# castorini/daam

Measured on NVIDIA H100. Metric: heatmap px/s (layers x steps x tokens), higher is better.
Workload: dtype bf16

## Files before the change

### daam_b200/csrc/accumulate_mma.cu

```cuda
#include <cuda.h>

#include <mutex>
#include <type_traits>
#include <unordered_map>
#include <string>

#include "common.cuh"

namespace daam {
namespace {

constexpr int kStages = 2;
constexpr int kAccStages = 3;
constexpr int kPrefetchTiles = 6;
constexpr int kQBytes = kTilePixels * 128;
constexpr int kKBytes = kTokensPad * 128;
constexpr int kStageBytes = kQBytes + kKBytes;
constexpr int kPBytes = kTokens * kTilePixels * 4;
constexpr int kConsumers = 256;
constexpr int kThreads = kConsumers + 32;
constexpr int kThreads16 = kConsumers + 64;
constexpr int kBarBytes = 64;
constexpr int kBarBytes16 = 8 * 2 * (kStages + kAccStages);
constexpr int kSmemBytes = 1024 + kStages * kStageBytes + kAccStages * kPBytes + kBarBytes16;
constexpr int kSlabSmemBytes = kSmemBytes + kPBytes;
constexpr int kSplitStageBytes = 2 * kStageBytes;
constexpr int kSplitSmemBytes = 1024 + (kStages + 1) * kSplitStageBytes + kPBytes + kBarBytes;
static_assert(kSmemBytes <= 232448, "16-bit form exceeds the 227 KB shared-memory limit");
static_assert(kSplitSmemBytes <= 232448, "split form exceeds the 227 KB shared-memory limit");
static_assert(kSlabSmemBytes <= 232448, "16-bit second-slab form exceeds the 227 KB shared-memory limit");
constexpr int long_smem_bytes(int chunks) {
  return 1024 + kStages * (kQBytes + chunks * kKBytes) + kAccStages * kPBytes + kBarBytes16;
}
static_assert(long_smem_bytes(3) <= 232448, "16-bit long-context form exceeds the 227 KB shared-memory limit");

struct MmaParams {
  LaunchParams base;
  CUtensorMap qmap[kMaxLayersPerLaunch];
  CUtensorMap kmap[kMaxLayersPerLaunch];
  CUtensorMap amap[kMaxLayersPerLaunch];
};
struct MmaSlabParams : MmaParams {
  CUtensorMap smap[kMaxLayersPerLaunch];
  float* slab[kMaxLayersPerLaunch];
};
template <bool kSecond>
using MmaParamsT = std::conditional_t<kSecond, MmaSlabParams, MmaParams>;

__device__ __forceinline__ uint32_t smem_u32(const void* p) { return (uint32_t)__cvta_generic_to_shared(p); }

__device__ __forceinline__ void mbar_init(uint32_t bar, uint32_t count) {
  asm volatile("mbarrier.init.shared::cta.b64 [%0], %1;" ::"r"(bar), "r"(count));
}
__device__ __forceinline__ void mbar_arrive(uint32_t bar) {
  asm volatile("mbarrier.arrive.shared::cta.b64 _, [%0];" ::"r"(bar) : "memory");
}
// ... 173 lines not shown
    for (int u = 0; u < 4; ++u)
      if (off + u * stride < end) {
        float4 h, l;
        h.x = trunc_tf32(x[u].x); h.y = trunc_tf32(x[u].y); h.z = trunc_tf32(x[u].z); h.w = trunc_tf32(x[u].w);
        l.x = rna_tf32(x[u].x - h.x); l.y = rna_tf32(x[u].y - h.y);
        l.z = rna_tf32(x[u].z - h.z); l.w = rna_tf32(x[u].w - h.w);
        *reinterpret_cast<float4*>(raw + off + u * stride) = h;
        *reinterpret_cast<float4*>(lo + off + u * stride) = l;
      }
  }
}

template <bool kBf16>
__device__ __forceinline__ void wgmma_chunk_16bit(Frag& d, uint32_t a_src, uint32_t k_src) {
  wgmma_fence();
#pragma unroll
  for (int k = 0; k < 4; ++k) wgmma_16bit<kBf16>(d, wgmma_desc_sw128(a_src + 32 * k), wgmma_desc_sw128(k_src + 32 * k));
  wgmma_commit();
  wgmma_wait0();
}
template <bool kBf16, int kC>
__device__ __forceinline__ void wgmma_chunk_16bit_long(Frag (&d)[kC], uint32_t a_src, uint32_t k_src) {
  wgmma_fence();
#pragma unroll
  for (int c = 0; c < kC; ++c)
#pragma unroll
    for (int k = 0; k < 4; ++k)
      wgmma_16bit<kBf16>(d[c], wgmma_desc_sw128(a_src + 32 * k), wgmma_desc_sw128(k_src + c * kKBytes + 32 * k));
  wgmma_commit();
  wgmma_wait0();
}

__device__ __forceinline__ void griddep_wait() { asm volatile("griddepcontrol.wait;" ::: "memory"); }

template <bool kSplit, bool kChunked, int kSlab, int kC = 1>
__global__ void __launch_bounds__(kSplit ? kThreads : kThreads16, 1)
accumulate_mma_kernel(const __grid_constant__ MmaParamsT<kSlab != kSlabNone> MP) {
  static_assert(kC == 1 || (!kSplit && kSlab == kSlabNone), "long contexts: 16-bit form, plain slab mode only");
  constexpr bool kSecond = kSlab != kSlabNone;
  constexpr int kCtx = kC * kTokens;
  constexpr int kStageBytesT = kSplit ? kSplitStageBytes : kQBytes + kC * kKBytes;
  constexpr int kOperandBytes = (kSplit ? kStages + 1 : kStages) * kStageBytesT;
  constexpr int kPTiles = kSplit ? 1 : kAccStages + (kSecond ? 1 : 0);
  const LaunchParams& P = MP.base;
  extern __shared__ uint8_t smem_raw[];
  const uint32_t raw = smem_u32(smem_raw);
  const uint32_t base = (raw + 1023u) & ~1023u;
  uint8_t* gen = smem_raw + (base - raw);
  float* sP = reinterpret_cast<float*>(gen + kOperandBytes);
  const uint32_t sP_u32 = base + kOperandBytes;
  float* sS = sP + kAccStages * (kTokens * kTilePixels);
  const uint32_t sS_u32 = sP_u32 + kAccStages * kPBytes;
  const uint32_t bars = sP_u32 + kPTiles * kPBytes;
  const uint32_t full0 = bars, empty0 = bars + 8 * kStages;
  const uint32_t afull0 = bars + 16 * kStages, aempty0 = afull0 + 8 * kAccStages;

  const int warp = threadIdx.x >> 5, lane = threadIdx.x & 31;
  int first, count, stride = 1;
  if constexpr (!kChunked && !kSplit) {
    first = blockIdx.x;
    stride = gridDim.x;
    count = (P.total_tiles - (int)blockIdx.x + stride - 1) / stride;
  } else if constexpr (!kChunked) {
    const int per = P.total_tiles / gridDim.x, rem = P.total_tiles % gridDim.x;
    first = blockIdx.x * per + min((int)blockIdx.x, rem);
    count = per + ((int)blockIdx.x < rem ? 1 : 0);
  } else {
    first = tile_at_weight(P, (long long)P.total_weight * blockIdx.x / gridDim.x);
    count = tile_at_weight(P, (long long)P.total_weight * (blockIdx.x + 1) / gridDim.x) - first;
  }

  if (threadIdx.x == 0) {
#pragma unroll
    for (int s = 0; s < kStages; ++s) {
      mbar_init(full0 + 8 * s, 1);
      mbar_init(empty0 + 8 * s, kConsumers / 32);
    }
    if constexpr (!kSplit) {
#pragma unroll
      for (int s = 0; s < kAccStages; ++s) {
        mbar_init(afull0 + 8 * s, 1);
        mbar_init(aempty0 + 8 * s, 1);
      }
    }
    asm volatile("fence.mbarrier_init.release.cluster;" ::: "memory");
  }
  if (count > 0 && lane == 0 && (warp == (kSplit ? 0 : 9) || warp == 8)) {
    int li0 = 0;
    const Tile t0 = decode_tile(P, first, li0);
    if (warp != 8) {
      prefetch_tensormap(&MP.amap[t0.li]);
      if constexpr (kSecond) prefetch_tensormap(&MP.smap[t0.li]);
    } else {
      prefetch_tensormap(&MP.qmap[t0.li]);
      prefetch_tensormap(&MP.kmap[t0.li]);
    }
  }
  __syncthreads();
  if (!P.early_loads) griddep_wait();
  asm volatile("griddepcontrol.launch_dependents;" ::: "memory");

  if (warp == 9) {
    if constexpr (!kSplit) {
      if (lane == 0 && count > 0) {
        if (P.early_loads) griddep_wait();
        const uint64_t pol = l2_evict_first();
        int li = 0;
        for (int i = 0; i < count; ++i) {
          const Tile t = decode_tile(P, first + i * stride, li);
#pragma unroll
          for (int c = 0; c < kC; ++c) {
            const int n = i * kC + c;
            const int a = n % kAccStages;
            mbar_wait(aempty0 + 8 * a, ((uint32_t)(n / kAccStages) & 1u) ^ 1u);
            mbar_expect_tx(afull0 + 8 * a, kPBytes);
            tma_load_2d_hint(&MP.amap[t.li], afull0 + 8 * a, sP_u32 + a * kPBytes, t.pixel0,
                             (t.prompt * P.layer[t.li].heads + t.head) * kCtx + c * kTokens, pol);
          }
        }
      }
    }
  } else if (warp == 8) {
    if (lane == 0) {
      int li = 0, j = 0;
      for (int i = 0; i < count; ++i) {
        if (!kSplit && P.early_loads && i == (kChunked ? 1 : kStages)) {
          const uint64_t pol = l2_evict_last();
          const int end = min(count, i + kPrefetchTiles);
          int pli = 0;
          Tile prev = decode_tile(P, first + (i - 1) * stride, pli);
          for (int p = i; p < end; ++p) {
            const Tile u = decode_tile(P, first + p * stride, pli);
            const bool new_head = u.li != prev.li || u.prompt != prev.prompt || u.head != prev.head;
            const int nc = kChunked ? (P.layer[u.li].head_dim + 63) >> 6 : 1;
            for (int c = 0; c < nc; ++c) {
              tma_prefetch_4d(&MP.qmap[u.li], 64 * c, u.head, u.pixel0, u.prompt, pol);
              if (new_head)
#pragma unroll
                for (int kc = 0; kc < kC; ++kc) tma_prefetch_4d(&MP.kmap[u.li], 64 * c, u.head, kc * kTokens, u.prompt, pol);
            }
            prev = u;
          }
        }
        const Tile t = decode_tile(P, first + i * stride, li);
        const int n_chunks = kChunked ? (P.layer[t.li].head_dim + 63) >> 6 : 1;
        for (int c = 0; c < n_chunks; ++c, ++j) {
          const int s = j % kStages;
          const uint32_t ph = (uint32_t)(j / kStages) & 1u;
          mbar_wait(empty0 + 8 * s, ph ^ 1u);
          const uint32_t q_dst = base + s * kStageBytesT;
          if constexpr (kSplit) {
// ... 101 lines not shown
        f[4 * jj + 2] = l0 ? fast_exp2(fmaf(f[4 * jj + 2], sc, -mc1)) : 0.f;
        f[4 * jj + 1] = l1 ? fast_exp2(fmaf(f[4 * jj + 1], sc, -mc0)) : 0.f;
        f[4 * jj + 3] = l1 ? fast_exp2(fmaf(f[4 * jj + 3], sc, -mc1)) : 0.f;
        sum0 += f[4 * jj] + f[4 * jj + 1];
        sum1 += f[4 * jj + 2] + f[4 * jj + 3];
      }
      sum0 += __shfl_xor_sync(0xffffffffu, sum0, 1);
      sum0 += __shfl_xor_sync(0xffffffffu, sum0, 2);
      sum1 += __shfl_xor_sync(0xffffffffu, sum1, 1);
      sum1 += __shfl_xor_sync(0xffffffffu, sum1, 2);
      const float inv0 = 1.0f / sum0, inv1 = 1.0f / sum1;

      if constexpr (!kSplit) {
#pragma unroll
        for (int kc = 0; kc < kC; ++kc) {
        const int n = i * kC + kc;
        const int a = n % kAccStages;
        float* sA = sP + a * (kTokens * kTilePixels);
        const bool lowq = quad < 2;
        const int ra = lowq ? r0 : r0 + 8, rb = lowq ? r0 + 8 : r0;
        mbar_wait(afull0 + 8 * a, (uint32_t)(n / kAccStages) & 1u);
        float old[40];
#pragma unroll
        for (int jj = 0; jj < 10; ++jj) {
#pragma unroll
          for (int e = 0; e < 2; ++e) {
            const int col = 8 * jj + 2 * quad + e;
            if (col < kTokens) {
              old[4 * jj + e] = sA[col * kTilePixels + ra];
              old[4 * jj + 2 + e] = sA[col * kTilePixels + rb];
            }
          }
        }
        if constexpr (kSecond) {
          if (tid == 0 && i > 0) bulk_wait_read0();
          consumer_barrier();
        }
        const float* f = dd[kc];
#pragma unroll
        for (int jj = 0; jj < 10; ++jj) {
#pragma unroll
          for (int e = 0; e < 2; ++e) {
            const int col = 8 * jj + 2 * quad + e;
            if (col < kTokens) {
              const float pa = f[4 * jj + e] * inv0, pb = f[4 * jj + 2 + e] * inv1;
              sA[col * kTilePixels + ra] = add_ftz(old[4 * jj + e], lowq ? pa : pb);
              sA[col * kTilePixels + rb] = add_ftz(old[4 * jj + 2 + e], lowq ? pb : pa);
              if constexpr (kSecond) {
                sS[col * kTilePixels + ra] = add_ftz(0.f, lowq ? pa : pb);
                sS[col * kTilePixels + rb] = add_ftz(0.f, lowq ? pb : pa);
              }
            }
          }
        }
        fence_proxy_async();
        consumer_barrier();
        if (tid == 0) {
          tma_store_2d_hint(&MP.amap[t.li], sP_u32 + a * kPBytes, t.pixel0,
                            (t.prompt * L.heads + t.head) * kCtx + kc * kTokens, l2_evict_first());
          if constexpr (kSlab == kSlabStore)
            tma_store_2d(&MP.smap[t.li], sS_u32, t.pixel0, (t.prompt * L.heads + t.head) * kTokens);
          if constexpr (kSlab == kSlabAdd)
            tma_reduce_add_2d(&MP.smap[t.li], sS_u32, t.pixel0, (t.prompt * L.heads + t.head) * kTokens);
          bulk_commit();
          if (n > 0) {
            bulk_wait_read1();
            mbar_arrive(aempty0 + 8 * ((n - 1) % kAccStages));
          }
        }
        }
        continue;
      }

      if (i == 0 && P.early_loads) griddep_wait();

      if (tid == 0 && issued) bulk_wait_read0();
      consumer_barrier();
      const bool lowq = quad < 2;
      const bool stage_ftz = kSlab == kSlabStore && P.rmw_mode == 1;
#pragma unroll
      for (int jj = 0; jj < 10; ++jj) {
#pragma unroll
        for (int e = 0; e < 2; ++e) {
          const int col = 8 * jj + 2 * quad + e;
          if (col < kTokens) {
            float a = d[4 * jj + e] * inv0, b = d[4 * jj + 2 + e] * inv1;
            if constexpr (kSecond) {
              if (stage_ftz) { a = add_ftz(0.f, a); b = add_ftz(0.f, b); }
            }
            sP[col * kTilePixels + (lowq ? r0 : r0 + 8)] = lowq ? a : b;
            sP[col * kTilePixels + (lowq ? r0 + 8 : r0)] = lowq ? b : a;
          }
        }
      }
      if (P.rmw_mode == 1) {
        fence_proxy_async();
        consumer_barrier();
        if (tid == 0) {
          tma_reduce_add_2d(&MP.amap[t.li], sP_u32, t.pixel0, (t.prompt * L.heads + t.head) * kTokens);
          if constexpr (kSlab == kSlabStore)
            tma_store_2d(&MP.smap[t.li], sP_u32, t.pixel0, (t.prompt * L.heads + t.head) * kTokens);
          if constexpr (kSlab == kSlabAdd)
            tma_reduce_add_2d(&MP.smap[t.li], sP_u32, t.pixel0, (t.prompt * L.heads + t.head) * kTokens);
          bulk_commit();
        }
        issued = true;
      } else {
        consumer_barrier();
        const long long hw = L.hw;
        float* acc = L.acc + ((long long)(t.prompt * L.heads + t.head) * kTokens) * hw + t.pixel0;
        const int live = min(kTilePixels, L.hw - t.pixel0) >> 2;
        for (int u = tid; u < kTokens * (kTilePixels / 4); u += kConsumers) {
          const int tok = u / (kTilePixels / 4), c4 = u % (kTilePixels / 4);
          if (c4 < live) {
            float4* g = reinterpret_cast<float4*>(acc + tok * hw) + c4;
            const float4 p = reinterpret_cast<const float4*>(sP + tok * kTilePixels)[c4];
            float4 o = *g;
            o.x += p.x; o.y += p.y; o.z += p.z; o.w += p.w;
            *g = o;
            if constexpr (kSlab == kSlabStore)
              reinterpret_cast<float4*>(MP.slab[t.li] + (acc - L.acc) + tok * hw)[c4] = p;
            if constexpr (kSlab == kSlabAdd) {
              float4* r = reinterpret_cast<float4*>(MP.slab[t.li] + (acc - L.acc) + tok * hw) + c4;
              float4 ro = *r;
              ro.x += p.x; ro.y += p.y; ro.z += p.z; ro.w += p.w;
              *r = ro;
            }
          }
        }
      }
    }
    if (tid == 0 && (kSplit ? issued : count > 0)) bulk_wait_read0();
  }
}

using EncodeFn = CUresult (*)(CUtensorMap*, CUtensorMapDataType, cuuint32_t, void*, const cuuint64_t*,
                              const cuuint64_t*, const cuuint32_t*, const cuuint32_t*, CUtensorMapInterleave,
                              CUtensorMapSwizzle, CUtensorMapL2promotion, CUtensorMapFloatOOBfill);

EncodeFn get_encode() {
  static EncodeFn fn = nullptr;
  static std::once_flag once;
  std::call_once(once, [] {
    void* p = nullptr;
    cudaDriverEntryPointQueryResult q;
    if (cudaGetDriverEntryPoint("cuTensorMapEncodeTiled", &p, cudaEnableDefault, &q) == cudaSuccess &&
        q == cudaDriverEntryPointSuccess)
      fn = reinterpret_cast<EncodeFn>(p);
  });
  return fn;
}

struct MapKey {
  const void* ptr;
  long long s1, s2, s3;
  int d1, d2, d3, kind;
  bool operator==(const MapKey& o) const {
    return ptr == o.ptr && s1 == o.s1 && s2 == o.s2 && s3 == o.s3 && d1 == o.d1 && d2 == o.d2 && d3 == o.d3 &&
           kind == o.kind;
  }
};
struct MapKeyHash {
  size_t operator()(const MapKey& k) const {
    size_t h = reinterpret_cast<size_t>(k.ptr);
    auto mix = [&h](long long v) { h ^= (size_t)v + 0x9e3779b97f4a7c15ull + (h << 6) + (h >> 2); };
// ... 113 lines not shown
    set_error("the wgmma kernel takes %d-token contexts, or 154 / 231 tokens for 16-bit layers without a second slab "
              "(got %d)", kTokens, ctx);
    return DAAM_E_UNSUPPORTED;
  }
  bool chunked = false;
  for (int i = 0; i < p.n_layers; ++i) {
    const LayerParams& L = p.layer[i];
    if ((L.dtype == DAAM_F32) != split) { set_error("mixed fp32 / 16-bit layers in one wgmma pack"); return DAAM_E_INVALID; }
    if (L.tokens != ctx) { set_error("mixed context lengths in one wgmma pack"); return DAAM_E_INVALID; }
    if (int rc = make_qk_map(L.q, L.dtype, L.head_dim, L.heads, L.hw, L.n_prompts, L.qs_head, L.qs_pixel, L.qs_prompt, kTilePixels, &mp.qmap[i])) return rc;
    if (int rc = make_qk_map(L.k, L.dtype, L.head_dim, L.heads, ctx, L.n_prompts, L.ks_head, L.ks_token, L.ks_prompt, kTokensPad, &mp.kmap[i])) return rc;
    if (int rc = make_acc_map(L.acc, L.hw, L.n_prompts * L.heads * ctx, &mp.amap[i])) return rc;
    if (slabs) {
      if (int rc = make_acc_map(slabs->slab[i], L.hw, L.n_prompts * L.heads * kTokens, &mp.smap[i])) return rc;
      mp.slab[i] = slabs->slab[i];
    }
    chunked = chunked || L.head_dim > 64;
  }
  cudaError_t attr_err = cudaSuccess;
  std::call_once(g_attr_once[dev.device & 63], [&] {
    for (const MmaInstance& k : kMmaInstances)
      if (cudaError_t e = cudaFuncSetAttribute(k.fn, cudaFuncAttributeMaxDynamicSharedMemorySize, k.smem)) attr_err = e;
  });
  DAAM_CUDA_TRY(attr_err);
  pm.grid = dev.sm_count;
  if (pm.grid > p.total_tiles) pm.grid = p.total_tiles;
  pm.block = split ? kThreads : kThreads16;
  pm.variant = ctx == kTokens ? (split ? 1 : 0) | (chunked ? 2 : 0) | (mode << 2)
                              : kLongVariant0 + (chunked ? 1 : 0) + (ctx == 3 * kTokens ? 2 : 0);
  pm.second = mode != kSlabNone;
  return DAAM_OK;
}

int launch_prepared_mma(const void* prepared, cudaStream_t stream) {
  const PreparedMma& pm = *static_cast<const PreparedMma*>(prepared);
  const MmaInstance& k = kMmaInstances[pm.variant];
  cudaLaunchConfig_t cfg = {};
  cfg.gridDim = dim3(pm.grid);
  cfg.blockDim = dim3(pm.block);
  cfg.dynamicSmemBytes = k.smem;
  cfg.stream = stream;
  cudaLaunchAttribute attr[1];
  attr[0].id = cudaLaunchAttributeProgrammaticStreamSerialization;
  attr[0].val.programmaticStreamSerializationAllowed = pm.mp.base.pdl ? 1 : 0;
  cfg.attrs = attr;
  cfg.numAttrs = 1;
  const MmaParams* plain = &pm.mp;
  void* args[] = {pm.second ? (void*)&pm.mp : (void*)plain};
  DAAM_CUDA_TRY(cudaLaunchKernelExC(&cfg, k.fn, args));
  DAAM_CUDA_TRY(cudaGetLastError());
  count_launch();
  return DAAM_OK;
}

}
```

### daam_b200/_native.py

```python
from __future__ import annotations

import ctypes
import os
from typing import Optional, Sequence, Tuple

LIB_NAME = 'libdaam_b200.so'
LIB_PATH = os.path.join(os.path.dirname(os.path.abspath(__file__)), LIB_NAME)

DAAM_F32, DAAM_F16, DAAM_BF16 = 0, 1, 2
ACC_AUTO, ACC_FORCE_SIMT, ACC_FORCE_MMA = 0, 1, 2
ACC_RMW_AUTO, ACC_RMW_LDST, ACC_RMW_RED = 0x00, 0x10, 0x20
ACC_NO_PDL = 0x100
ACC_EARLY_LOADS = 0x200
ABI_VERSION = 4
E_INVALID, E_UNSUPPORTED, E_CUDA = -1, -2, -3
TOKENS = 77
CONTEXT_TOKENS = (77, 154, 231)
EXPAND_SCRATCH_FLOATS = 64
MAX_SEGMENT_WORDS = 96


def segment_scratch_floats(n_maps: int, n_words: int) -> int:
    return 64 * n_maps * n_words

# ... 6 lines not shown

SWEEP_MAX_THRESHOLDS = 64


def region_sweep_scratch_floats(n_maps: int, n_words: int, n_regions: int, n_thresholds: int, out_h: int,
                                out_w: int) -> int:
    return n_maps * n_words * (64 + (n_regions + 1) * n_thresholds)


WORD_OVERLAP_CTAS = 256


def word_overlap_scratch_floats(n_maps: int, n_words: int, out_h: int, out_w: int) -> int:
    tiles = ((out_h + 15) // 16) * ((out_w + 63) // 64)
    return n_maps * (n_words * 64 + (n_words * (n_words + 3) // 2) * min(tiles, WORD_OVERLAP_CTAS))


WORD_INSTANCES_MAX = 64


def word_instances_plane_bytes(out_h: int, out_w: int) -> int:
    return 8 * out_h * out_w + 48 * ((out_h + 1) // 2) * ((out_w + 1) // 2) + 260


def overlay_frames_bytes(n_maps: int, n_words: int, out_h: int, out_w: int) -> int:
    return (n_maps * n_words * out_h * out_w * 3 + 3) // 4 * 4


EXPORTS = ('daam_accumulate', 'daam_accumulate_steps', 'daam_accumulate_range', 'daam_attention_probs', 'daam_accumulate_probs', 'daam_finalize',
           'daam_finalize_maps', 'daam_finalize_parts', 'daam_finalize_per_key','daam_normalize_maps', 'daam_word_heat_map', 'daam_expand_as', 'daam_expand_words',
           'daam_segment_words', 'daam_region_overlap', 'daam_region_sweep', 'daam_word_overlap', 'daam_word_instances', 'daam_overlay_words', 'daam_jet_colormap',
           'daam_side_launcher_create', 'daam_side_launcher_destroy',
           'daam_side_launcher_launch', 'daam_side_launcher_join', 'daam_side_launcher_idle', 'daam_abi_version',
           'daam_last_error', 'daam_device_info', 'daam_launch_count')


class DaamLayer(ctypes.Structure):
    _fields_ = [
        ('q', ctypes.c_void_p), ('k', ctypes.c_void_p), ('acc', ctypes.c_void_p),
        ('q_stride_prompt', ctypes.c_int64), ('q_stride_pixel', ctypes.c_int64), ('q_stride_head', ctypes.c_int64),
        ('k_stride_prompt', ctypes.c_int64), ('k_stride_token', ctypes.c_int64), ('k_stride_head', ctypes.c_int64),
        ('n_prompts', ctypes.c_int32), ('heads', ctypes.c_int32), ('hw', ctypes.c_int32), ('tokens', ctypes.c_int32),
        ('head_dim', ctypes.c_int32), ('dtype', ctypes.c_int32), ('scale', ctypes.c_float),
        ('reserved', ctypes.c_int32),
    ]


class DaamKeyGroup(ctypes.Structure):
    _fields_ = [
        ('acc', ctypes.c_void_p), ('heads', ctypes.c_int32), ('h', ctypes.c_int32), ('w', ctypes.c_int32),
        ('tokens', ctypes.c_int32), ('head_sel', ctypes.c_int32), ('n_blocks', ctypes.c_int32),
    ]
    reserved = property(lambda self: self.n_blocks, lambda self, v: setattr(self, 'n_blocks', v))


class DaamMapSel(ctypes.Structure):
    _fields_ = [
        ('block_begin', ctypes.c_int32), ('block_count', ctypes.c_int32), ('n_rows', ctypes.c_int32),
        ('reserved', ctypes.c_int32), ('out', ctypes.c_void_p),
    ]


class DaamMapPart(ctypes.Structure):
    _fields_ = [
        ('group_begin', ctypes.c_int32), ('group_count', ctypes.c_int32), ('n_rows', ctypes.c_int32),
        ('reserved', ctypes.c_int32), ('out', ctypes.c_void_p),
    ]
# ... 61 lines not shown
    lib.daam_region_overlap.argtypes = [vp, i32, i32, i32, i32, ctypes.POINTER(i32), ctypes.POINTER(i32), i32, i32, i32,
                                        i32, i32, f32, vp, vp, i32, vp, vp, vp, vp]
    lib.daam_region_overlap.restype = ctypes.c_int
    lib.daam_region_sweep.argtypes = [vp, i32, i32, i32, i32, ctypes.POINTER(i32), ctypes.POINTER(i32), i32, i32, i32,
                                      i32, ctypes.POINTER(f32), i32, vp, vp, i32, vp, vp, vp, vp]
    lib.daam_region_sweep.restype = ctypes.c_int
    lib.daam_word_overlap.argtypes = [vp, i32, i32, i32, i32, ctypes.POINTER(i32), ctypes.POINTER(i32), i32, i32, i32,
                                      i32, i32, f32, vp, vp, vp, vp, vp]
    lib.daam_word_overlap.restype = ctypes.c_int
    lib.daam_word_instances.argtypes = [vp, i32, i32, i32, i32, ctypes.POINTER(i32), ctypes.POINTER(i32), i32, i32,
                                        i32, i32, f32, i32, vp, vp, vp, vp, vp, vp, vp, vp, i64, vp]
    lib.daam_word_instances.restype = ctypes.c_int
    lib.daam_overlay_words.argtypes = [vp, i32, i32, i32, i32, ctypes.POINTER(i32), ctypes.POINTER(i32), i32, i32, i32,
                                       i32, i32, f32, i32, vp, vp, i64, vp, vp, vp]
    lib.daam_overlay_words.restype = ctypes.c_int
    lib.daam_jet_colormap.argtypes = [vp]
    lib.daam_jet_colormap.restype = ctypes.c_int
    lib.daam_side_launcher_create.argtypes = [ctypes.POINTER(vp)]
    lib.daam_side_launcher_create.restype = ctypes.c_int
    lib.daam_side_launcher_destroy.argtypes = [vp]
    lib.daam_side_launcher_destroy.restype = None
    lib.daam_side_launcher_launch.argtypes = [vp, ctypes.POINTER(DaamLayer), i32, u32, vp, vp]
    lib.daam_side_launcher_launch.restype = ctypes.c_int
    lib.daam_side_launcher_join.argtypes = [vp, vp]
    lib.daam_side_launcher_join.restype = ctypes.c_int
    lib.daam_side_launcher_idle.argtypes = [vp]
    lib.daam_side_launcher_idle.restype = ctypes.c_int
    lib.daam_last_error.argtypes = []
    lib.daam_last_error.restype = ctypes.c_char_p
    lib.daam_device_info.argtypes = [ctypes.POINTER(i32)] * 3
    lib.daam_device_info.restype = ctypes.c_int
    lib.daam_launch_count.argtypes = []
    lib.daam_launch_count.restype = i64
    _lib = lib
    return lib


def _check(rc: int):
    if rc != 0:
        raise NativeError(rc, load().daam_last_error().decode('utf-8', 'replace'))


class PackedLayers:

    def __init__(self, layers: Sequence[DaamLayer]):
        self.n = len(layers)
        self.array = (DaamLayer * max(self.n, 1))(*layers)


class SideLauncher:

    def __init__(self):
        self._lib = load()
        handle = ctypes.c_void_p()
        _check(self._lib.daam_side_launcher_create(ctypes.byref(handle)))
        self._h = handle

    def launch(self, packed: 'PackedLayers', flags: int, producer_stream: int, side_stream: int):
        rc = self._lib.daam_side_launcher_launch(self._h, packed.array, packed.n, flags, producer_stream, side_stream)
        if rc != 0:
            _check(rc)

    def join(self, stream: int):
        rc = self._lib.daam_side_launcher_join(self._h, stream)
        if rc != 0:
            _check(rc)
# ... 202 lines not shown
                                      *_word_list(x, rows_per_word, out_h, out_w, absolute, threshold)[:-2],
                                      float(threshold), max_instances, vp(word_maps_ptr), vp(count_ptr), vp(area_ptr),
                                      vp(box_ptr), vp(sum_yx_ptr), vp(peak_ptr), vp(peak_yx_ptr), vp(scratch_ptr),
                                      scratch_bytes, vp(stream)))


def overlay_words(maps_ptr: int, n_maps: int, n_rows: int, x, rows_per_word: Sequence[Sequence[int]], out_h: int,
                  out_w: int, absolute: bool, threshold: Optional[float], color_normalize: bool, word_maps_ptr: int,
                  image_ptr: int, image_map_stride: int, frames_ptr: int, scratch_ptr: int, stream: int):
    _check(load().daam_overlay_words(ctypes.c_void_p(maps_ptr), n_maps, n_rows,
                                     *_word_list(x, rows_per_word, out_h, out_w, absolute, threshold),
                                     int(bool(color_normalize)), ctypes.c_void_p(word_maps_ptr),
                                     ctypes.c_void_p(image_ptr), image_map_stride, ctypes.c_void_p(frames_ptr),
                                     ctypes.c_void_p(scratch_ptr), ctypes.c_void_p(stream)))


def jet_colormap():
    import torch
    out = torch.empty((256, 3), dtype=torch.float32)
    _check(load().daam_jet_colormap(ctypes.c_void_p(out.data_ptr())))
    return out


def device_info():
    sm, major, minor = ctypes.c_int32(), ctypes.c_int32(), ctypes.c_int32()
    _check(load().daam_device_info(ctypes.byref(sm), ctypes.byref(major), ctypes.byref(minor)))
    return {'sm_count': sm.value, 'cc': (major.value, minor.value)}


def launch_count() -> int:
    return int(load().daam_launch_count())


def abi_version() -> int:
    return int(load().daam_abi_version())
```

### daam_b200/csrc/api.cu

```cuda
#include <atomic>
#include <cstdarg>
#include <cstdio>
#include <cstring>
#include <memory>
#include <mutex>
#include <vector>

#include "common.cuh"

namespace daam {

static thread_local char g_error[512] = "";
static std::atomic<long long> g_launches{0};

void set_error(const char* fmt, ...) {
  va_list ap;
  va_start(ap, fmt);
  vsnprintf(g_error, sizeof(g_error), fmt, ap);
  va_end(ap);
}

int cuda_fail(cudaError_t e, const char* what) {
  set_error("CUDA error %d (%s) in %s", (int)e, cudaGetErrorString(e), what);
  return DAAM_E_CUDA;
}

void count_launch(int n) { g_launches.fetch_add(n, std::memory_order_relaxed); }

int get_device_info(DeviceInfo* out) {
  static std::mutex mu;
  static DeviceInfo cache[64];
  int dev = 0;
  DAAM_CUDA_TRY(cudaGetDevice(&dev));
  std::lock_guard<std::mutex> lock(mu);
  if (dev < 0 || dev >= 64) { set_error("device index %d out of range", dev); return DAAM_E_CUDA; }
  if (cache[dev].device != dev) {
    cudaDeviceProp prop;
    DAAM_CUDA_TRY(cudaGetDeviceProperties(&prop, dev));
// ... 14 lines not shown
  if (in.dtype != DAAM_F32 && in.dtype != DAAM_F16 && in.dtype != DAAM_BF16) { set_error("daam_accumulate: layer %d: unknown dtype %d", index, in.dtype); return DAAM_E_INVALID; }
  if (in.tokens != kTokens && in.tokens != 2 * kTokens && in.tokens != 3 * kTokens) { set_error("daam_accumulate: layer %d: tokens = %d, only %d, %d or %d (one to three %d-token CLIP chunks) are traced", index, in.tokens, kTokens, 2 * kTokens, 3 * kTokens, kTokens); return DAAM_E_UNSUPPORTED; }
  if (in.head_dim <= 0 || in.head_dim % 8 != 0 || in.head_dim > DAAM_MAX_HEAD_DIM) { set_error("daam_accumulate: layer %d: head_dim = %d must be a multiple of 8 in (0, %d]", index, in.head_dim, DAAM_MAX_HEAD_DIM); return DAAM_E_UNSUPPORTED; }
  if (in.n_prompts <= 0 || in.heads <= 0 || in.hw <= 0) { set_error("daam_accumulate: layer %d: non-positive n_prompts/heads/hw", index); return DAAM_E_INVALID; }
  if (need_acc && reinterpret_cast<uintptr_t>(in.acc) % 16 != 0) { set_error("daam_accumulate: layer %d: acc is not 16-byte aligned", index); return DAAM_E_INVALID; }
  if (!(in.scale > 0.f)) { set_error("daam_accumulate: layer %d: scale must be positive", index); return DAAM_E_INVALID; }
  LayerParams& L = *out;
  L.q = in.q; L.k = in.k; L.acc = in.acc;
  L.qs_prompt = in.q_stride_prompt; L.qs_pixel = in.q_stride_pixel; L.qs_head = in.q_stride_head;
  L.ks_prompt = in.k_stride_prompt; L.ks_token = in.k_stride_token; L.ks_head = in.k_stride_head;
  L.n_prompts = in.n_prompts; L.heads = in.heads; L.hw = in.hw; L.head_dim = in.head_dim;
  L.dtype = in.dtype;
  L.scale_log2e = in.scale * 1.4426950408889634f;
  L.tiles_per_head = (in.hw + kTilePixels - 1) / kTilePixels;
  L.tile_begin = 0;
  const size_t es = dtype_size(in.dtype);
  auto aligned = [&](long long stride) { return (stride * (long long)es) % 16 == 0; };
  L.weight = 1;
  L.weight_begin = 0;
  L.vec_ok = reinterpret_cast<uintptr_t>(in.q) % 16 == 0 && reinterpret_cast<uintptr_t>(in.k) % 16 == 0 &&
             aligned(in.q_stride_prompt) && aligned(in.q_stride_pixel) && aligned(in.q_stride_head) &&
             aligned(in.k_stride_prompt) && aligned(in.k_stride_token) && aligned(in.k_stride_head);
  L.tokens = in.tokens;
  return DAAM_OK;
}

}

using namespace daam;

namespace daam {
namespace {

struct PlannedLaunch {
  bool is_mma = false;
  LaunchParams simt;
  SlabMode mode = kSlabNone;
  SecondSlabs slabs;
  int grid = 0;
  size_t smem = 0;
  struct MmaDeleter { void operator()(void* p) const { prepared_mma_delete(p); } };
  std::unique_ptr<void, MmaDeleter> mma;
};

struct Plan {
  std::vector<uint8_t> key;
  uint32_t flags = 0;
  int device = -1;
  SlabMode mode = kSlabNone;
  std::vector<PlannedLaunch> launches;
  uint64_t stamp = 0;
};
constexpr size_t kMaxPlans = 32;

size_t slab_bytes(const LayerParams& l) { return (size_t)l.n_prompts * l.heads * l.tokens * l.hw * sizeof(float); }

bool spans_overlap(const void* a, size_t na, const void* b, size_t nb) {
  const char *pa = static_cast<const char*>(a), *pb = static_cast<const char*>(b);
  return pa < pb + nb && pb < pa + na;
}

bool acc_overlap(const LayerParams& a, const LayerParams& b) {
  return spans_overlap(a.acc, slab_bytes(a), b.acc, slab_bytes(b));
}

const char* slab_word(SlabMode mode) { return mode == kSlabAdd ? "range" : "step"; }

int validate_second_slabs(const char* fn, const daam_layer* layers, float* const* slabs, int n_layers, SlabMode mode) {
// ... 5 lines not shown
  }
  for (int i = 0; i < n_layers; ++i) {
    if (!slabs[i]) { set_error("%s: layer %d has a null %s slab", fn, i, what); return DAAM_E_INVALID; }
    if (reinterpret_cast<uintptr_t>(slabs[i]) % 16 != 0) { set_error("%s: layer %d: the %s slab is not 16-byte aligned", fn, i, what); return DAAM_E_INVALID; }
  }
  for (int i = 0; i < n_layers; ++i) {
    const size_t n = slab_bytes(all[i]);
    for (int j = 0; j < n_layers; ++j) {
      if (spans_overlap(slabs[i], n, all[j].acc, slab_bytes(all[j]))) {
        set_error("%s: the %s slab of layer %d overlaps the accumulator of layer %d", fn, what, i, j);
        return DAAM_E_INVALID;
      }
      if (j != i && spans_overlap(slabs[i], n, slabs[j], slab_bytes(all[j]))) {
        set_error("%s: the %s slabs of layers %d and %d overlap", fn, what, i, j);
        return DAAM_E_INVALID;
      }
    }
  }
  return DAAM_OK;
}

int build_plan(const daam_layer* layers, float* const* slabs, SlabMode mode, int n_layers, uint32_t flags,
               const DeviceInfo& dev, Plan* plan) {
  const uint32_t path = flags & 3u, rmw = flags & DAAM_ACC_RMW_MASK;
  constexpr int kPacks = 7;
  LaunchParams packs[kPacks];
  SecondSlabs pack_slabs[kPacks];
  for (LaunchParams& p : packs) {
    p.n_layers = p.total_tiles = 0;
    p.rmw_mode = (rmw == DAAM_ACC_RMW_LDST) ? 0 : 1;
    p.pdl = (flags & DAAM_ACC_NO_PDL) ? 0 : 1;
    p.early_loads = (flags & DAAM_ACC_EARLY_LOADS) && p.pdl ? 1 : 0;
    p.total_weight = 0;
  }
  packs[1].early_loads = 0;
  auto close = [&](int which) -> int {
    LaunchParams& p = packs[which];
    if (p.n_layers == 0) return DAAM_OK;
    plan->launches.emplace_back();
    PlannedLaunch& l = plan->launches.back();
    l.is_mma = which != 2 && which < 5;
    const SecondSlabs* st = slabs ? &pack_slabs[which] : nullptr;
    int rc;
    if (l.is_mma) {
      l.mma.reset(prepared_mma_new());
      rc = prepare_accumulate_mma(p, st, mode, dev, l.mma.get());
    } else {
      l.simt = p;
      l.mode = mode;
      if (st) l.slabs = *st;
      rc = prepare_accumulate_simt(p, mode, dev, &l.grid, &l.smem);
    }
    p.n_layers = 0;
    p.total_tiles = 0;
    p.total_weight = 0;
    return rc;
  };
  for (int i = 0; i < n_layers; ++i) {
    LayerParams L;
    if (int rc = make_layer_params(layers[i], i, &L, true)) return rc;
    const int ctx_chunks = L.tokens / kTokens;
    const bool use_mma = path != DAAM_ACC_FORCE_SIMT && dev.cc_major == 9 && mma_supported(L) &&
                         (ctx_chunks == 1 || L.dtype != DAAM_F32);
    if (path == DAAM_ACC_FORCE_MMA && !use_mma) {
      set_error("daam_accumulate: layer %d cannot take the wgmma path (dtype %d, head_dim %d, alignment %d, hw = %d, "
                "tokens = %d, %d prompts with prompt strides q %lld / k %lld, sm_%d%d)", i, L.dtype, L.head_dim,
                L.vec_ok, L.hw, L.tokens, L.n_prompts, L.qs_prompt, L.ks_prompt, dev.cc_major, dev.cc_minor);
      return DAAM_E_UNSUPPORTED;
    }
    const int which = ctx_chunks > 1 ? (use_mma ? 1 : 3) + ctx_chunks : use_mma ? (L.dtype == DAAM_F32 ? 1 : 0) : 2;
    LaunchParams& p = packs[which];
    for (int m = 0; m < p.n_layers; ++m)
      if (acc_overlap(p.layer[m], L)) {
        if (int rc = close(which)) return rc;
        break;
      }
    L.tile_begin = p.total_tiles;
    const int n_chunks = (L.head_dim + 63) / 64;
    L.weight = which == 1 ? n_chunks : 1 + 4 * n_chunks;
    L.weight_begin = p.total_weight;
    if (slabs) pack_slabs[which].slab[p.n_layers] = slabs[i];
    p.layer[p.n_layers++] = L;
    p.total_tiles += L.tiles_per_head * L.heads * L.n_prompts;
    p.total_weight += L.tiles_per_head * L.heads * L.n_prompts * L.weight;
    if (p.n_layers == kMaxLayersPerLaunch)
      if (int rc = close(which)) return rc;
  }
  for (int which = 0; which < kPacks; ++which)
    if (int rc = close(which)) return rc;
  return DAAM_OK;
}

}
}

namespace daam {
namespace {

int accumulate_impl(const char* fn, const daam_layer* layers, float* const* slabs, SlabMode mode, int32_t n_layers,
                    uint32_t flags, void* stream_) {
  if (n_layers < 0 || (n_layers > 0 && !layers)) { set_error("%s: bad layer array", fn); return DAAM_E_INVALID; }
  if (n_layers == 0) return DAAM_OK;
  const bool with_slabs = mode != kSlabNone;
  if (with_slabs && !slabs) { set_error("%s: %s_acc is a null array", fn, slab_word(mode)); return DAAM_E_INVALID; }
  cudaStream_t stream = static_cast<cudaStream_t>(stream_);
  DeviceInfo dev;
  if (int rc = get_device_info(&dev)) return rc;

  static thread_local std::vector<std::unique_ptr<Plan>> plans;
  static thread_local uint64_t clock = 0;
  const size_t layer_bytes = sizeof(daam_layer) * (size_t)n_layers;
  const size_t slab_ptr_bytes = with_slabs ? sizeof(float*) * (size_t)n_layers : 0;
  const size_t bytes = layer_bytes + slab_ptr_bytes;
  Plan* plan = nullptr;
  for (auto& c : plans)
    if (c->key.size() == bytes && c->flags == flags && c->device == dev.device && c->mode == mode &&
        memcmp(c->key.data(), layers, layer_bytes) == 0 &&
        (!with_slabs || memcmp(c->key.data() + layer_bytes, slabs, slab_ptr_bytes) == 0)) {
      plan = c.get();
      break;
    }
  if (!plan) {
    if (with_slabs)
      if (int rc = validate_second_slabs(fn, layers, slabs, n_layers, mode)) return rc;
    std::unique_ptr<Plan> fresh(new Plan);
    fresh->key.assign(reinterpret_cast<const uint8_t*>(layers), reinterpret_cast<const uint8_t*>(layers) + layer_bytes);
    if (with_slabs)
      fresh->key.insert(fresh->key.end(), reinterpret_cast<const uint8_t*>(slabs),
                        reinterpret_cast<const uint8_t*>(slabs) + slab_ptr_bytes);
    fresh->flags = flags;
    fresh->device = dev.device;
    fresh->mode = mode;
    if (int rc = build_plan(layers, slabs, mode, n_layers, flags, dev, fresh.get())) return rc;
    if (plans.size() >= kMaxPlans) {
      size_t oldest = 0;
      for (size_t i = 1; i < plans.size(); ++i)
        if (plans[i]->stamp < plans[oldest]->stamp) oldest = i;
      plans[oldest] = std::move(fresh);
      plan = plans[oldest].get();
    } else {
      plans.push_back(std::move(fresh));
      plan = plans.back().get();
    }
  }
  plan->stamp = ++clock;
  for (const PlannedLaunch& l : plan->launches) {
    const int rc = l.is_mma ? launch_prepared_mma(l.mma.get(), stream)
                            : launch_prepared_simt(l.simt, l.mode != kSlabNone ? &l.slabs : nullptr, l.mode, l.grid,
                                                   l.smem, stream);
    if (rc) return rc;
  }
  return DAAM_OK;
}

}
}

extern "C" int daam_accumulate(const daam_layer* layers, int32_t n_layers, uint32_t flags, void* stream) {
  return accumulate_impl("daam_accumulate", layers, nullptr, kSlabNone, n_layers, flags, stream);
}

extern "C" int daam_accumulate_steps(const daam_layer* layers, float* const* step_acc, int32_t n_layers, uint32_t flags,
                                     void* stream) {
  return accumulate_impl("daam_accumulate_steps", layers, step_acc, kSlabStore, n_layers, flags, stream);
}

extern "C" int daam_accumulate_range(const daam_layer* layers, float* const* range_acc, int32_t n_layers, uint32_t flags,
                                     void* stream) {
  return accumulate_impl("daam_accumulate_range", layers, range_acc, kSlabAdd, n_layers, flags, stream);
}

struct daam_side_launcher {
  cudaEvent_t ready = nullptr, done = nullptr;
  int device = -1;
  bool launched = false;
};

extern "C" int daam_side_launcher_create(daam_side_launcher** out) {
  if (!out) { set_error("daam_side_launcher_create: null pointer"); return DAAM_E_INVALID; }
  DeviceInfo dev;
  if (int rc = get_device_info(&dev)) return rc;
  std::unique_ptr<daam_side_launcher> h(new daam_side_launcher);
  h->device = dev.device;
  DAAM_CUDA_TRY(cudaEventCreateWithFlags(&h->ready, cudaEventDisableTiming));
// ... 12 lines not shown
  delete h;
}

extern "C" int daam_side_launcher_launch(daam_side_launcher* h, const daam_layer* layers, int32_t n_layers, uint32_t flags,
                                         void* producer_stream, void* side_stream) {
  if (!h) { set_error("daam_side_launcher_launch: null launcher"); return DAAM_E_INVALID; }
  cudaStream_t producer = static_cast<cudaStream_t>(producer_stream), side = static_cast<cudaStream_t>(side_stream);
  DAAM_CUDA_TRY(cudaEventRecord(h->ready, producer));
  DAAM_CUDA_TRY(cudaStreamWaitEvent(side, h->ready, 0));
  if (int rc = daam_accumulate(layers, n_layers, flags, side_stream)) return rc;
  DAAM_CUDA_TRY(cudaEventRecord(h->done, side));
  h->launched = true;
  return DAAM_OK;
}

extern "C" int daam_side_launcher_join(daam_side_launcher* h, void* stream) {
  if (!h) { set_error("daam_side_launcher_join: null launcher"); return DAAM_E_INVALID; }
  if (h->launched) DAAM_CUDA_TRY(cudaStreamWaitEvent(static_cast<cudaStream_t>(stream), h->done, 0));
  return DAAM_OK;
}

extern "C" int daam_side_launcher_idle(daam_side_launcher* h) {
  if (!h) { set_error("daam_side_launcher_idle: null launcher"); return DAAM_E_INVALID; }
  if (!h->launched) return 1;
  const cudaError_t e = cudaEventQuery(h->done);
  if (e == cudaSuccess) return 1;
  if (e == cudaErrorNotReady) return 0;
  return cuda_fail(e, "cudaEventQuery");
}

extern "C" int daam_abi_version(void) { return DAAM_ABI_VERSION; }
extern "C" const char* daam_last_error(void) { return g_error; }
extern "C" int64_t daam_launch_count(void) { return g_launches.load(std::memory_order_relaxed); }

extern "C" int daam_device_info(int32_t* sm_count, int32_t* cc_major, int32_t* cc_minor) {
  DeviceInfo dev;
  if (int rc = get_device_info(&dev)) return rc;
  if (sm_count) *sm_count = dev.sm_count;
  if (cc_major) *cc_major = dev.cc_major;
  if (cc_minor) *cc_minor = dev.cc_minor;
  return DAAM_OK;
}
```

### daam_b200/csrc/common.cuh

```cuda
#pragma once

#include <cuda_runtime.h>
#include <cuda_bf16.h>
#include <cuda_fp16.h>
#include <stdint.h>

#include "daam_b200.h"

namespace daam {

constexpr int kTokens = DAAM_TOKENS;
constexpr int kTokensPad = 80;
constexpr int kTilePixels = 128;
constexpr int kMaxLayersPerLaunch = 32;

struct LayerParams {
  const void* q;
  const void* k;
  float* acc;
  long long qs_prompt, qs_pixel, qs_head;
  long long ks_prompt, ks_token, ks_head;
  int n_prompts, heads, hw, head_dim;
  int dtype;
  float scale_log2e;
  int tiles_per_head;
  int tile_begin;
  int vec_ok;
  int weight;
  int weight_begin;
  int tokens;
};

struct LaunchParams {
  int n_layers;
  int total_tiles;
  int rmw_mode;
  int pdl;
  int early_loads;
  int total_weight;
  LayerParams layer[kMaxLayersPerLaunch];
};

__device__ __forceinline__ float fast_exp2(float x) {
  float y;
  asm("ex2.approx.ftz.f32 %0, %1;" : "=f"(y) : "f"(x));
  return y;
}

__device__ __forceinline__ float add_ftz(float a, float b) {
  float r;
  asm("add.rn.ftz.f32 %0, %1, %2;" : "=f"(r) : "f"(a), "f"(b));
  return r;
}

struct SecondSlabs {
  float* slab[kMaxLayersPerLaunch];
};
enum SlabMode : int { kSlabNone = 0, kSlabStore = 1, kSlabAdd = 2 };

void set_error(const char* fmt, ...);
int cuda_fail(cudaError_t e, const char* what);
#define DAAM_CUDA_TRY(expr)                                        \
  do {                                                             \
    cudaError_t e_ = (expr);                                       \
    if (e_ != cudaSuccess) return ::daam::cuda_fail(e_, #expr);    \
  } while (0)

struct DeviceInfo {
  int device = -1;
  int sm_count = 0;
  int cc_major = 0, cc_minor = 0;
};
int get_device_info(DeviceInfo* out);
void count_launch(int n = 1);

int prepare_accumulate_simt(const LaunchParams& p, SlabMode mode, const DeviceInfo& dev, int* grid, size_t* smem);
int launch_prepared_simt(const LaunchParams& p, const SecondSlabs* slabs, SlabMode mode, int grid, size_t smem,
                         cudaStream_t stream);
void* prepared_mma_new();
void prepared_mma_delete(void* prepared);
int prepare_accumulate_mma(const LaunchParams& p, const SecondSlabs* slabs, SlabMode mode, const DeviceInfo& dev,
                           void* prepared);
int launch_prepared_mma(const void* prepared, cudaStream_t stream);
bool mma_supported(const LayerParams& l);

}
```

### include/daam_b200.h

```cpp
#ifndef DAAM_B200_H
#define DAAM_B200_H

#include <stdint.h>

#ifdef __cplusplus
extern "C" {
#endif

#define DAAM_ABI_VERSION 4
#define DAAM_TOKENS 77
#define DAAM_MAX_TOKENS 231
#define DAAM_MAX_HEAD_DIM 256

enum daam_status {
  DAAM_OK = 0,
  DAAM_E_INVALID = -1,
  DAAM_E_UNSUPPORTED = -2,
  DAAM_E_CUDA = -3
};

enum daam_dtype { DAAM_F32 = 0, DAAM_F16 = 1, DAAM_BF16 = 2 };

#define DAAM_ACC_AUTO        0u
#define DAAM_ACC_FORCE_SIMT  1u
// ... 109 lines not shown
#define DAAM_WORD_OVERLAP_CTAS 256
#define DAAM_WORD_OVERLAP_SCRATCH_FLOATS(n_maps, n_words, out_h, out_w)                                               \
  ((int64_t)(n_maps) * ((n_words) * 64 + ((n_words) * ((n_words) + 3) / 2) *                                         \
       ((((out_h) + 15) / 16) * (((out_w) + 63) / 64) < DAAM_WORD_OVERLAP_CTAS                                       \
            ? (((out_h) + 15) / 16) * (((out_w) + 63) / 64) : DAAM_WORD_OVERLAP_CTAS)))
int daam_word_overlap(const float* global_maps, int32_t n_maps, int32_t n_rows, int32_t map_h, int32_t map_w,
                      const int32_t* rows, const int32_t* row_begin, int32_t n_words, int32_t out_h, int32_t out_w,
                      int32_t absolute, int32_t use_threshold, float threshold, float* word_maps,
                      float* intersection, float* word_area, float* scratch, void* stream);

#define DAAM_WORD_INSTANCES_MAX 64
#define DAAM_WORD_INSTANCES_PLANE_BYTES(out_h, out_w)                                                                 \
  (8 * (int64_t)(out_h) * (out_w) + 48 * (int64_t)(((out_h) + 1) / 2) * (((out_w) + 1) / 2) + 260)
int daam_word_instances(const float* global_maps, int32_t n_maps, int32_t n_rows, int32_t map_h, int32_t map_w,
                        const int32_t* rows, const int32_t* row_begin, int32_t n_words, int32_t out_h, int32_t out_w,
                        int32_t absolute, float threshold, int32_t max_instances, float* word_maps, int32_t* count,
                        int32_t* area, int32_t* box, int64_t* sum_yx, float* peak, int32_t* peak_yx, void* scratch,
                        int64_t scratch_bytes, void* stream);

#define DAAM_OVERLAY_FRAMES_BYTES(n_maps, n_words, out_h, out_w)                                                      \
  (((int64_t)(n_maps) * (n_words) * (out_h) * (out_w) * 3 + 3) / 4 * 4)
int daam_overlay_words(const float* global_maps, int32_t n_maps, int32_t n_rows, int32_t map_h, int32_t map_w,
                       const int32_t* rows, const int32_t* row_begin, int32_t n_words, int32_t out_h, int32_t out_w,
                       int32_t absolute, int32_t use_threshold, float threshold, int32_t color_normalize,
                       float* word_maps, const uint8_t* image, int64_t image_map_stride, uint8_t* frames,
                       float* scratch, void* stream);

int daam_jet_colormap(float* out);

int daam_abi_version(void);
const char* daam_last_error(void);
int daam_device_info(int32_t* sm_count, int32_t* cc_major, int32_t* cc_minor);
int64_t daam_launch_count(void);

#ifdef __cplusplus
}
#endif
#endif
```

Before: 267.5 billion.

## Move accumulator TMA stores to a dedicated store warp with mbarrier handoff

Adds a third producer-side warp that waits on new per-stage 'filled' mbarriers and issues the TMA stores and slab stores and reductions, then frees accumulator stages. Consumers no longer run a block-wide barrier and single-thread store issue after each tile; each warp just arrives on the barrier. This aims to take store issue and bulk-wait latency off the consumer critical path. It costs an extra warp and more barriers, and adds subtle phase and ordering logic around the shared slab buffer (sfree) that could introduce races.

```diff
diff --git a/daam_b200/csrc/accumulate_mma.cu b/daam_b200/csrc/accumulate_mma.cu
--- a/daam_b200/csrc/accumulate_mma.cu
+++ b/daam_b200/csrc/accumulate_mma.cu
@@ -19,9 +19,9 @@
 constexpr int kPBytes = kTokens * kTilePixels * 4;
 constexpr int kConsumers = 256;
 constexpr int kThreads = kConsumers + 32;
-constexpr int kThreads16 = kConsumers + 64;
+constexpr int kThreads16 = kConsumers + 96;
 constexpr int kBarBytes = 64;
-constexpr int kBarBytes16 = 8 * 2 * (kStages + kAccStages);
+constexpr int kBarBytes16 = 8 * (2 * kStages + 3 * kAccStages + 1);
 constexpr int kSmemBytes = 1024 + kStages * kStageBytes + kAccStages * kPBytes + kBarBytes16;
 constexpr int kSlabSmemBytes = kSmemBytes + kPBytes;
 constexpr int kSplitStageBytes = 2 * kStageBytes;
@@ -283,6 +283,8 @@
   const uint32_t bars = sP_u32 + kPTiles * kPBytes;
   const uint32_t full0 = bars, empty0 = bars + 8 * kStages;
   const uint32_t afull0 = bars + 16 * kStages, aempty0 = afull0 + 8 * kAccStages;
+  const uint32_t afilled0 = aempty0 + 8 * kAccStages;
+  const uint32_t sfree = afilled0 + 8 * kAccStages;
 
   const int warp = threadIdx.x >> 5, lane = threadIdx.x & 31;
   int first, count, stride = 1;
@@ -310,7 +312,9 @@
       for (int s = 0; s < kAccStages; ++s) {
         mbar_init(afull0 + 8 * s, 1);
         mbar_init(aempty0 + 8 * s, 1);
-      }
+        mbar_init(afilled0 + 8 * s, kConsumers / 32);
+      }
+      mbar_init(sfree, 1);
     }
     asm volatile("fence.mbarrier_init.release.cluster;" ::: "memory");
   }
@@ -329,7 +333,52 @@
   if (!P.early_loads) griddep_wait();
   asm volatile("griddepcontrol.launch_dependents;" ::: "memory");
 
-  if (warp == 9) {
+  if (warp == 10) {
+    if constexpr (!kSplit) {
+      if (lane == 0 && count > 0) {
+        const uint64_t pol = l2_evict_first();
+        int li = 0;
+        bool held = false;
+        Tile t = decode_tile(P, first, li);
+        for (int i = 0; i < count; ++i) {
+          Tile next = t;
+          if (i + 1 < count) {
+            next = decode_tile(P, first + (i + 1) * stride, li);
+            if (next.li != t.li) {
+              prefetch_tensormap(&MP.amap[next.li]);
+              if constexpr (kSecond) prefetch_tensormap(&MP.smap[next.li]);
+            }
+          }
+          const int row = t.prompt * P.layer[t.li].heads + t.head;
+#pragma unroll
+          for (int c = 0; c < kC; ++c) {
+            const int n = i * kC + c;
+            const int a = n % kAccStages;
+            mbar_wait(afilled0 + 8 * a, (uint32_t)(n / kAccStages) & 1u);
+            tma_store_2d_hint(&MP.amap[t.li], sP_u32 + a * kPBytes, t.pixel0, row * kCtx + c * kTokens, pol);
+            if constexpr (kSlab == kSlabStore)
+              tma_store_2d(&MP.smap[t.li], sS_u32, t.pixel0, row * kTokens);
+            if constexpr (kSlab == kSlabAdd)
+              tma_reduce_add_2d(&MP.smap[t.li], sS_u32, t.pixel0, row * kTokens);
+            bulk_commit();
+            if (held) {
+              bulk_wait_read1();
+              mbar_arrive(aempty0 + 8 * ((n - 1) % kAccStages));
+              if constexpr (kSecond) mbar_arrive(sfree);
+            }
+            const int n1 = n + 1;
+            held = n1 < count * kC && mbar_try(afilled0 + 8 * (n1 % kAccStages), (uint32_t)(n1 / kAccStages) & 1u);
+            if (!held) {
+              bulk_wait_read0();
+              mbar_arrive(aempty0 + 8 * a);
+              if constexpr (kSecond) mbar_arrive(sfree);
+            }
+          }
+          t = next;
+        }
+      }
+    }
+  } else if (warp == 9) {
     if constexpr (!kSplit) {
       if (lane == 0 && count > 0) {
         if (P.early_loads) griddep_wait();
@@ -513,10 +562,8 @@
             }
           }
         }
-        if constexpr (kSecond) {
-          if (tid == 0 && i > 0) bulk_wait_read0();
-          consumer_barrier();
-        }
+        if constexpr (kSecond)
+          mbar_wait(sfree, ((uint32_t)i & 1u) ^ 1u);
         const float* f = dd[kc];
 #pragma unroll
         for (int jj = 0; jj < 10; ++jj) {
@@ -535,20 +582,8 @@
           }
         }
         fence_proxy_async();
-        consumer_barrier();
-        if (tid == 0) {
-          tma_store_2d_hint(&MP.amap[t.li], sP_u32 + a * kPBytes, t.pixel0,
-                            (t.prompt * L.heads + t.head) * kCtx + kc * kTokens, l2_evict_first());
-          if constexpr (kSlab == kSlabStore)
-            tma_store_2d(&MP.smap[t.li], sS_u32, t.pixel0, (t.prompt * L.heads + t.head) * kTokens);
-          if constexpr (kSlab == kSlabAdd)
-            tma_reduce_add_2d(&MP.smap[t.li], sS_u32, t.pixel0, (t.prompt * L.heads + t.head) * kTokens);
-          bulk_commit();
-          if (n > 0) {
-            bulk_wait_read1();
-            mbar_arrive(aempty0 + 8 * ((n - 1) % kAccStages));
-          }
-        }
+        __syncwarp();
+        if (lane == 0) mbar_arrive(afilled0 + 8 * a);
         }
         continue;
       }
@@ -611,7 +646,7 @@
         }
       }
     }
-    if (tid == 0 && (kSplit ? issued : count > 0)) bulk_wait_read0();
+    if (tid == 0 && issued) bulk_wait_read0();
   }
 }
 
```

Measured after the change: 267.2 billion (median of 6 runs). About the same (-0.1%).

## Defer PDL grid-dependency wait when consecutive launches touch disjoint accumulators

Applied to the files above, without the earlier changes.

Tracks the accumulator address spans written by the previous launch on each stream at host level. When the next MMA launch uses early loads and its spans do not overlap, it skips the initial griddepcontrol.wait and lets the producer warp issue the first kAccStages accumulator TMA loads before waiting, so it overlaps more with the prior kernel's tail. The launch_dependents trigger is also moved to sit after the wait. This adds host mutex and map bookkeeping per launch plus a capture query, and relies on the span-disjointness reasoning being correct. It only applies when early loads are enabled and the stream is not being captured.

```diff
diff --git a/daam_b200/_native.py b/daam_b200/_native.py
--- a/daam_b200/_native.py
+++ b/daam_b200/_native.py
@@ -62,7 +62,7 @@
            'daam_segment_words', 'daam_region_overlap', 'daam_region_sweep', 'daam_word_overlap', 'daam_word_instances', 'daam_overlay_words', 'daam_jet_colormap',
            'daam_side_launcher_create', 'daam_side_launcher_destroy',
            'daam_side_launcher_launch', 'daam_side_launcher_join', 'daam_side_launcher_idle', 'daam_abi_version',
-           'daam_last_error', 'daam_device_info', 'daam_launch_count')
+           'daam_last_error', 'daam_device_info', 'daam_launch_count', 'daam_acc_free_count')
 
 
 class DaamLayer(ctypes.Structure):
@@ -190,6 +190,8 @@
     lib.daam_device_info.restype = ctypes.c_int
     lib.daam_launch_count.argtypes = []
     lib.daam_launch_count.restype = i64
+    lib.daam_acc_free_count.argtypes = []
+    lib.daam_acc_free_count.restype = i64
     _lib = lib
     return lib
 
@@ -458,5 +460,9 @@
     return int(load().daam_launch_count())
 
 
+def acc_free_count() -> int:
+    return int(load().daam_acc_free_count())
+
+
 def abi_version() -> int:
     return int(load().daam_abi_version())
diff --git a/daam_b200/csrc/accumulate_mma.cu b/daam_b200/csrc/accumulate_mma.cu
--- a/daam_b200/csrc/accumulate_mma.cu
+++ b/daam_b200/csrc/accumulate_mma.cu
@@ -261,6 +261,9 @@
 }
 
 __device__ __forceinline__ void griddep_wait() { asm volatile("griddepcontrol.wait;" ::: "memory"); }
+__device__ __forceinline__ void griddep_launch_dependents() {
+  asm volatile("griddepcontrol.launch_dependents;" ::: "memory");
+}
 
 template <bool kSplit, bool kChunked, int kSlab, int kC = 1>
 __global__ void __launch_bounds__(kSplit ? kThreads : kThreads16, 1)
@@ -326,13 +329,20 @@
     }
   }
   __syncthreads();
-  if (!P.early_loads) griddep_wait();
-  asm volatile("griddepcontrol.launch_dependents;" ::: "memory");
+  if (!P.early_loads) {
+    griddep_wait();
+    griddep_launch_dependents();
+  }
 
   if (warp == 9) {
     if constexpr (!kSplit) {
-      if (lane == 0 && count > 0) {
-        if (P.early_loads) griddep_wait();
+      if (lane == 0) {
+        bool waited = !P.early_loads;
+        if (!waited && !P.acc_free) {
+          griddep_wait();
+          griddep_launch_dependents();
+          waited = true;
+        }
         const uint64_t pol = l2_evict_first();
         int li = 0;
         for (int i = 0; i < count; ++i) {
@@ -341,11 +351,20 @@
           for (int c = 0; c < kC; ++c) {
             const int n = i * kC + c;
             const int a = n % kAccStages;
+            if (!waited && n == kAccStages) {
+              griddep_wait();
+              griddep_launch_dependents();
+              waited = true;
+            }
             mbar_wait(aempty0 + 8 * a, ((uint32_t)(n / kAccStages) & 1u) ^ 1u);
             mbar_expect_tx(afull0 + 8 * a, kPBytes);
             tma_load_2d_hint(&MP.amap[t.li], afull0 + 8 * a, sP_u32 + a * kPBytes, t.pixel0,
                              (t.prompt * P.layer[t.li].heads + t.head) * kCtx + c * kTokens, pol);
           }
+        }
+        if (!waited) {
+          griddep_wait();
+          griddep_launch_dependents();
         }
       }
     }
@@ -791,9 +810,10 @@
   return DAAM_OK;
 }
 
-int launch_prepared_mma(const void* prepared, cudaStream_t stream) {
-  const PreparedMma& pm = *static_cast<const PreparedMma*>(prepared);
+int launch_prepared_mma(void* prepared, bool acc_free, cudaStream_t stream) {
+  PreparedMma& pm = *static_cast<PreparedMma*>(prepared);
   const MmaInstance& k = kMmaInstances[pm.variant];
+  pm.mp.base.acc_free = acc_free ? 1 : 0;
   cudaLaunchConfig_t cfg = {};
   cfg.gridDim = dim3(pm.grid);
   cfg.blockDim = dim3(pm.block);
diff --git a/daam_b200/csrc/api.cu b/daam_b200/csrc/api.cu
--- a/daam_b200/csrc/api.cu
+++ b/daam_b200/csrc/api.cu
@@ -1,9 +1,12 @@
+#include <algorithm>
 #include <atomic>
 #include <cstdarg>
 #include <cstdio>
 #include <cstring>
+#include <map>
 #include <memory>
 #include <mutex>
+#include <utility>
 #include <vector>
 
 #include "common.cuh"
@@ -84,8 +87,14 @@
 namespace daam {
 namespace {
 
+struct Span {
+  uintptr_t lo, hi;
+};
+
 struct PlannedLaunch {
   bool is_mma = false;
+  bool tracked = false;
+  std::vector<Span> spans;
   LaunchParams simt;
   SlabMode mode = kSlabNone;
   SecondSlabs slabs;
@@ -157,6 +166,7 @@
     p.pdl = (flags & DAAM_ACC_NO_PDL) ? 0 : 1;
     p.early_loads = (flags & DAAM_ACC_EARLY_LOADS) && p.pdl ? 1 : 0;
     p.total_weight = 0;
+    p.acc_free = 0;
   }
   packs[1].early_loads = 0;
   auto close = [&](int which) -> int {
@@ -166,6 +176,13 @@
     PlannedLaunch& l = plan->launches.back();
     l.is_mma = which != 2 && which < 5;
     const SecondSlabs* st = slabs ? &pack_slabs[which] : nullptr;
+    l.tracked = l.is_mma && which != 1 && p.early_loads && mode == kSlabNone;
+    for (int m = 0; m < p.n_layers; ++m) {
+      const uintptr_t a = reinterpret_cast<uintptr_t>(p.layer[m].acc), n = slab_bytes(p.layer[m]);
+      l.spans.push_back({a, a + n});
+      if (st) l.spans.push_back({reinterpret_cast<uintptr_t>(st->slab[m]), reinterpret_cast<uintptr_t>(st->slab[m]) + n});
+    }
+    std::sort(l.spans.begin(), l.spans.end(), [](const Span& x, const Span& y) { return x.lo < y.lo; });
     int rc;
     if (l.is_mma) {
       l.mma.reset(prepared_mma_new());
@@ -221,6 +238,43 @@
 
 namespace daam {
 namespace {
+
+std::mutex g_records_mu;
+std::map<std::pair<int, cudaStream_t>, std::vector<Span>> g_records;
+std::atomic<long long> g_acc_free_launches{0};
+
+bool lists_overlap(const std::vector<Span>& a, const std::vector<Span>& b) {
+  size_t i = 0, j = 0;
+  while (i < a.size() && j < b.size()) {
+    if (a[i].hi <= b[j].lo) ++i;
+    else if (b[j].hi <= a[i].lo) ++j;
+    else return true;
+  }
+  return false;
+}
+
+int launch_planned(PlannedLaunch& l, int device, cudaStream_t stream, bool capturing) {
+  if (stream == cudaStreamLegacy) stream = nullptr;
+  const bool trackable = stream != cudaStreamPerThread && !capturing;
+  std::lock_guard<std::mutex> lock(g_records_mu);
+  const auto key = std::make_pair(device, stream);
+  auto it = g_records.find(key);
+  int rc;
+  if (l.is_mma) {
+    const bool acc_free = l.tracked && trackable && it != g_records.end() && !lists_overlap(it->second, l.spans);
+    rc = launch_prepared_mma(l.mma.get(), acc_free, stream);
+    if (!rc && acc_free) g_acc_free_launches.fetch_add(1, std::memory_order_relaxed);
+  } else {
+    rc = launch_prepared_simt(l.simt, l.mode != kSlabNone ? &l.slabs : nullptr, l.mode, l.grid, l.smem, stream);
+  }
+  if (!rc && l.tracked && trackable) {
+    if (it == g_records.end()) it = g_records.emplace(key, std::vector<Span>()).first;
+    it->second.assign(l.spans.begin(), l.spans.end());
+  } else if (it != g_records.end()) {
+    g_records.erase(it);
+  }
+  return rc;
+}
 
 int accumulate_impl(const char* fn, const daam_layer* layers, float* const* slabs, SlabMode mode, int32_t n_layers,
                     uint32_t flags, void* stream_) {
@@ -269,12 +323,12 @@
     }
   }
   plan->stamp = ++clock;
-  for (const PlannedLaunch& l : plan->launches) {
-    const int rc = l.is_mma ? launch_prepared_mma(l.mma.get(), stream)
-                            : launch_prepared_simt(l.simt, l.mode != kSlabNone ? &l.slabs : nullptr, l.mode, l.grid,
-                                                   l.smem, stream);
-    if (rc) return rc;
-  }
+  cudaStreamCaptureStatus capture = cudaStreamCaptureStatusNone;
+  const cudaError_t query = cudaStreamIsCapturing(stream, &capture);
+  if (query != cudaSuccess) (void)cudaGetLastError();
+  const bool capturing = query != cudaSuccess || capture != cudaStreamCaptureStatusNone;
+  for (PlannedLaunch& l : plan->launches)
+    if (int rc = launch_planned(l, dev.device, stream, capturing)) return rc;
   return DAAM_OK;
 }
 
@@ -353,6 +407,7 @@
 extern "C" int daam_abi_version(void) { return DAAM_ABI_VERSION; }
 extern "C" const char* daam_last_error(void) { return g_error; }
 extern "C" int64_t daam_launch_count(void) { return g_launches.load(std::memory_order_relaxed); }
+extern "C" int64_t daam_acc_free_count(void) { return g_acc_free_launches.load(std::memory_order_relaxed); }
 
 extern "C" int daam_device_info(int32_t* sm_count, int32_t* cc_major, int32_t* cc_minor) {
   DeviceInfo dev;
diff --git a/daam_b200/csrc/common.cuh b/daam_b200/csrc/common.cuh
--- a/daam_b200/csrc/common.cuh
+++ b/daam_b200/csrc/common.cuh
@@ -38,6 +38,7 @@
   int pdl;
   int early_loads;
   int total_weight;
+  int acc_free;
   LayerParams layer[kMaxLayersPerLaunch];
 };
 
@@ -81,7 +82,7 @@
 void prepared_mma_delete(void* prepared);
 int prepare_accumulate_mma(const LaunchParams& p, const SecondSlabs* slabs, SlabMode mode, const DeviceInfo& dev,
                            void* prepared);
-int launch_prepared_mma(const void* prepared, cudaStream_t stream);
+int launch_prepared_mma(void* prepared, bool acc_free, cudaStream_t stream);
 bool mma_supported(const LayerParams& l);
 
 }
diff --git a/include/daam_b200.h b/include/daam_b200.h
--- a/include/daam_b200.h
+++ b/include/daam_b200.h
@@ -165,6 +165,7 @@
 const char* daam_last_error(void);
 int daam_device_info(int32_t* sm_count, int32_t* cc_major, int32_t* cc_minor);
 int64_t daam_launch_count(void);
+int64_t daam_acc_free_count(void);
 
 #ifdef __cplusplus
 }
```

Result: faster. 266.5 billion before, 271.2 billion after, median of 6 (+1.7%).
